# aerius-labs/paillier-halo2

Hardware: AMD Instinct MI355X
Metric: Paillier-encrypt proofs/s (2048-bit n, k=17); MSM achieved HBM GB/s vs peak (higher is better)
Workload: dtype u32 limbs (29-bit reduced radix, 254-bit modular integers), u64 limbs (4096-bit integers)

## Files before the change

### paillier_halo2_amd/csrc/pz_quotient.hip

```cpp
#include "fp29.cuh"
#include "pz_internal.h"

static inline Fr fp_one_host() {
    static const uint64_t ONE[4] = {0xac96341c4ffffffbULL, 0x36fc76959f60cd29ULL, 0x666ea36f7879462eULL, 0x0e0a77c19a07df2fULL};
    Fr r;
    memcpy(r.v, ONE, 32);
    return r;
}
static inline Fr fr_from_u64(const uint64_t x[4]) {
    Fr r;
    memcpy(r.v, x, 32);
    return r;
}

typedef F29<FrTag> Fr29;
__device__ __forceinline__ Fr29 fr29_c261(const Fr& c) { return f29_to_261(f29_from_fp(c)); }
__device__ __forceinline__ Fr29 fr29_one256() {
    Fr29 r;
#pragma unroll
    for (int i = 0; i < 9; ++i) r.v[i] = P29<FrTag>::R256(i);
    return r;
}

struct S29 {
    u32 v[9];
};
static bool host_fr_canonical(const uint64_t c[4]) {
    static const uint64_t R[4] = {0x43e1f593f0000001ULL, 0x2833e84879b97091ULL, 0xb85045b68181585dULL, 0x30644e72e131a029ULL};
    for (int i = 3; i >= 0; --i)
        if (c[i] != R[i]) return c[i] < R[i];
    return false;
}
static S29 host_fr_shl(const uint64_t c[4], unsigned k) {
    static const uint64_t R[4] = {0x43e1f593f0000001ULL, 0x2833e84879b97091ULL, 0xb85045b68181585dULL, 0x30644e72e131a029ULL};
    uint64_t x[4] = {c[0], c[1], c[2], c[3]};
    for (unsigned t = 0; t < k; ++t) {
        for (int i = 3; i > 0; --i) x[i] = (x[i] << 1) | (x[i - 1] >> 63);
        x[0] <<= 1;
        bool ge = true;
        for (int i = 3; i >= 0; --i)
            if (x[i] != R[i]) { ge = x[i] > R[i]; break; }
        if (ge) {
            unsigned __int128 br = 0;
            for (int i = 0; i < 4; ++i) {
                const unsigned __int128 d = (unsigned __int128)x[i] - R[i] - br;
                x[i] = (uint64_t)d;
                br = (d >> 64) & 1;
            }
        }
    }
    S29 r;
    for (int i = 0; i < 9; ++i) {
        const unsigned bit = 29u * i, j = bit >> 6, o = bit & 63;
        uint64_t w = x[j] >> o;
        if (o > 35 && j + 1 < 4) w |= x[j + 1] << (64 - o);
        r.v[i] = (u32)(w & (i < 8 ? 0x1fffffffull : 0xffffffffull));
    }
    return r;
}
static void host_fr_mul(const uint64_t a[4], const uint64_t b[4], uint64_t out[4]) {
    static const uint64_t R[4] = {0x43e1f593f0000001ULL, 0x2833e84879b97091ULL, 0xb85045b68181585dULL, 0x30644e72e131a029ULL};
    const uint64_t INV = 0xc2e1f593efffffffULL;
    uint64_t t[6] = {0, 0, 0, 0, 0, 0};
    for (int i = 0; i < 4; ++i) {
        unsigned __int128 c = 0;
        for (int j = 0; j < 4; ++j) {
            c += (unsigned __int128)a[j] * b[i] + t[j];
            t[j] = (uint64_t)c;
            c >>= 64;
        }
        c += t[4];
        t[4] = (uint64_t)c;
        t[5] = (uint64_t)(c >> 64);
        const uint64_t m = t[0] * INV;
        c = ((unsigned __int128)m * R[0] + t[0]) >> 64;
        for (int j = 1; j < 4; ++j) {
            c += (unsigned __int128)m * R[j] + t[j];
            t[j - 1] = (uint64_t)c;
            c >>= 64;
        }
        c += t[4];
        t[3] = (uint64_t)c;
        t[4] = t[5] + (uint64_t)(c >> 64);
    }
    bool ge = t[4] != 0;
    if (!ge) {
        ge = true;
        for (int i = 3; i >= 0; --i)
            if (t[i] != R[i]) { ge = t[i] > R[i]; break; }
    }
    if (ge) {
        unsigned __int128 br = 0;
        for (int i = 0; i < 4; ++i) {
            const unsigned __int128 d = (unsigned __int128)t[i] - R[i] - br;
            t[i] = (uint64_t)d;
            br = (d >> 64) & 1;
        }
    }
    memcpy(out, t, 32);
}
static void host_fr_pow(const uint64_t a[4], unsigned e, uint64_t out[4]) {
    static const uint64_t ONE[4] = {0xac96341c4ffffffbULL, 0x36fc76959f60cd29ULL, 0x666ea36f7879462eULL, 0x0e0a77c19a07df2fULL};
    uint64_t acc[4], sq[4];
    memcpy(acc, ONE, 32);
    memcpy(sq, a, 32);
    for (; e; e >>= 1) {
        if (e & 1) host_fr_mul(acc, sq, acc);
        host_fr_mul(sq, sq, sq);
    }
    memcpy(out, acc, 32);
}
extern "C" int pzx_host_selftest(void) {
    static const uint64_t ONE[4] = {0xac96341c4ffffffbULL, 0x36fc76959f60cd29ULL, 0x666ea36f7879462eULL, 0x0e0a77c19a07df2fULL};
    auto limbs_of = [](const uint64_t x[4]) { return host_fr_shl(x, 0); };
    auto same = [](const S29& a, const S29& b) { return memcmp(a.v, b.v, sizeof a.v) == 0; };
    uint64_t two[4], acc[4], pw[4];
    {
        const S29 d = host_fr_shl(ONE, 1);
        unsigned __int128 carry = 0;
        memset(two, 0, sizeof two);
        for (int i = 0; i < 9; ++i) {
            const unsigned bit = 29u * i, j = bit >> 6, o = bit & 63;
            two[j] |= (uint64_t)d.v[i] << o;
            if (o > 35 && j + 1 < 4) two[j + 1] |= (uint64_t)d.v[i] >> (64 - o);
        }
        (void)carry;
    }
    if (!same(limbs_of(two), host_fr_shl(ONE, 1))) return 1;
    host_fr_mul(ONE, ONE, acc);
    if (memcmp(acc, ONE, 32)) return 2;
    memcpy(acc, ONE, 32);
    for (unsigned k = 1; k <= 300; ++k) {
        host_fr_mul(acc, two, acc);
        if (!same(limbs_of(acc), host_fr_shl(ONE, k))) return 100 + (int)k;
        if (k % 37 == 0 || k == 300) {
            host_fr_pow(two, k, pw);
            if (memcmp(pw, acc, 32)) return 1000 + (int)k;
        }
    }
    return 0;
}
extern "C" void pzx_host_fr_mul(const uint64_t a[4], const uint64_t b[4], uint64_t out[4]) { host_fr_mul(a, b, out); }
extern "C" void pzx_host_fr_pow(const uint64_t a[4], unsigned e, uint64_t out[4]) { host_fr_pow(a, e, out); }
extern "C" void pzx_host_fr_shl(const uint64_t c[4], unsigned k, uint32_t out[9]) {
    const S29 r = host_fr_shl(c, k);
    memcpy(out, r.v, sizeof r.v);
}
__device__ __forceinline__ Fr29 f29_add_s(const Fr29& a, const u32 (&b)[9]) {
    Fr29 r;
#pragma unroll
    for (int i = 0; i < 9; ++i) r.v[i] = a.v[i] + b[i];
    return r;
}

__global__ __launch_bounds__(256) void k_batch_invert(Fr* __restrict__ a, Fr* __restrict__ scratch, size_t n, size_t T,
                                                      unsigned K, Fr* __restrict__ mul_io) {
    const size_t t = (size_t)blockIdx.x * blockDim.x + threadIdx.x;
    if (t >= T) return;
    Fr29 acc = fr29_one256();
    for (unsigned j = 0; j < K; ++j) {
        const size_t i = t + (size_t)j * T;
        if (i >= n) break;
        const Fr v = fp_load<FrTag>(a + i);
        if (fp_is_zero(v)) continue;
        Fr w;
        f29_pack(acc, w.v);
        fp_store(scratch + i, w);
        acc = f29_mul(acc, f29_from_fp_shl5(v));
    }
    Fr29 inv = f29_mul(f29_inv(acc), fr29_one256());
    for (unsigned j = K; j-- > 0;) {
        const size_t i = t + (size_t)j * T;
        if (i >= n) continue;
        const Fr v = fp_load<FrTag>(a + i);
        if (fp_is_zero(v)) {
            if (mul_io) fp_store(mul_io + i, fp_zero<FrTag>());
            continue;
        }
        const Fr29 ai = f29_mul(inv, f29_load<FrTag>(scratch + i));
        if (mul_io) f29_store_product(mul_io + i, f29_mul(ai, f29_load_shl5<FrTag>(mul_io + i)));
        else f29_store_product(a + i, ai);
        inv = f29_mul(inv, f29_from_fp_shl5(v));
    }
}

int pz_batch_invert_internal(pz_ctx* ctx, Fr* d_a, size_t n, Fr* d_mul_io) {
    if (!n) return PZ_OK;
    void* scr;
    PZCHK(pz_ws_get(ctx, WS_BIG_A, n * 32, &scr));
    unsigned K = 8;
    while (K < 64 && n / (K * 2) >= 16384) K *= 2;
    while (K < 512 && n / (K * 2) >= 262144) K *= 2;
    const size_t T = pz_div_up(n, K);
    hipLaunchKernelGGL(k_batch_invert, dim3(pz_div_up(T, 256)), dim3(256), 0, ctx->stream, d_a, (Fr*)scr, n, T, K, d_mul_io);
    HIPCHK(ctx, hipGetLastError());
    return PZ_OK;
}

extern "C" int pz_fr_batch_invert_dev(pz_ctx* ctx, uint64_t* d_a, size_t n) {
    if (!ctx || (n && !d_a)) return PZ_ERR_INVALID;
    PZ_ENTER(ctx);
    return pz_batch_invert_internal(ctx, (Fr*)d_a, n, nullptr);
}

#define PP_K 16u
__global__ __launch_bounds__(256) void k_pp_local(const Fr* __restrict__ a, size_t as, size_t n, Fr* __restrict__ excl,
                                                  Fr* __restrict__ block_tot, unsigned nb) {
    __shared__ u32 s[9 * 256];
    a += (size_t)blockIdx.y * as;
    const size_t t = (size_t)blockIdx.x * 256 + threadIdx.x;
    const size_t lo = t * PP_K;
    Fr29 p = fr29_one256();
    for (unsigned j = 0; j < PP_K; ++j)
        if (lo + j < n) p = f29_mul(p, f29_load_shl5<FrTag>(a + lo + j));
    p = f29_to_261(p);
#pragma unroll
    for (int i = 0; i < 9; ++i) s[i * 256 + threadIdx.x] = p.v[i];
    __syncthreads();
    for (unsigned off = 1; off < 256; off <<= 1) {
        Fr29 u;
        if (threadIdx.x >= off) {
#pragma unroll
            for (int i = 0; i < 9; ++i) u.v[i] = s[i * 256 + threadIdx.x - off];
        }
        __syncthreads();
        if (threadIdx.x >= off) {
            p = f29_mul(u, p);
#pragma unroll
            for (int i = 0; i < 9; ++i) s[i * 256 + threadIdx.x] = p.v[i];
        }
        __syncthreads();
    }
    Fr29 e = f29_one<FrTag>();
    if (threadIdx.x) {
#pragma unroll
        for (int i = 0; i < 9; ++i) e.v[i] = s[i * 256 + threadIdx.x - 1];
    }
    Fr w;
    f29_pack(e, w.v);
    fp_store(excl + (size_t)blockIdx.y * nb * 256 + t, w);
    if (threadIdx.x == 255) f29_store_product(block_tot + (size_t)blockIdx.y * nb + blockIdx.x, f29_to_256(p));
}
__global__ void k_pp_blocks(Fr* __restrict__ block_tot, unsigned nb, size_t n_cols, Fr z0) {
    const size_t col = (size_t)blockIdx.x * blockDim.x + threadIdx.x;
    if (col >= n_cols) return;
    Fr* bt = block_tot + col * nb;
    Fr run = z0;
    for (unsigned b = 0; b < nb; ++b) {
        Fr t = fp_load<FrTag>(bt + b);
        fp_store(bt + b, run);
        run = fp_mul(run, t);
    }
}
__global__ __launch_bounds__(256) void k_pp_apply(const Fr* __restrict__ a, size_t as, size_t n, const Fr* __restrict__ excl,
                                                  const Fr* __restrict__ block_tot, unsigned nb, Fr* __restrict__ z, size_t zs) {
    a += (size_t)blockIdx.y * as;
    z += (size_t)blockIdx.y * zs;
    const size_t t = (size_t)blockIdx.x * 256 + threadIdx.x;
    const size_t lo = t * PP_K;
    if (lo >= n) return;
    Fr29 cur = f29_mul(f29_load<FrTag>(block_tot + (size_t)blockIdx.y * nb + blockIdx.x),
                       f29_load<FrTag>(excl + (size_t)blockIdx.y * nb * 256 + t));
    for (unsigned j = 0; j < PP_K && lo + j < n; ++j) {
        const Fr v = fp_load<FrTag>(a + lo + j);
        f29_store_product(z + lo + j, cur);
        cur = f29_mul(cur, f29_from_fp_shl5(v));
    }
}

int pz_prefix_product_batch_internal(pz_ctx* ctx, const Fr* d_a, size_t a_stride, size_t n_cols, size_t n, Fr z0, Fr* d_z,
                                     size_t z_stride) {
    if (!n || !n_cols) return PZ_OK;
    if (n_cols > 65535) return PZ_ERR_INVALID;
    const unsigned nb = pz_div_up(pz_div_up(n, PP_K), 256);
    void* ws;
    PZCHK(pz_ws_get(ctx, WS_BIG_B, n_cols * ((size_t)nb * 256 + nb) * 32, &ws));
    Fr* excl = (Fr*)ws;
    Fr* tot = excl + n_cols * (size_t)nb * 256;
    hipLaunchKernelGGL(k_pp_local, dim3(nb, (unsigned)n_cols), dim3(256), 0, ctx->stream, d_a, a_stride, n, excl, tot, nb);
    hipLaunchKernelGGL(k_pp_blocks, dim3(pz_div_up(n_cols, 64)), dim3(64), 0, ctx->stream, tot, nb, n_cols, z0);
    hipLaunchKernelGGL(k_pp_apply, dim3(nb, (unsigned)n_cols), dim3(256), 0, ctx->stream, d_a, a_stride, n, (const Fr*)excl,
                       (const Fr*)tot, nb, d_z, z_stride);
    HIPCHK(ctx, hipGetLastError());
    return PZ_OK;
}
int pz_prefix_product_internal(pz_ctx* ctx, const Fr* d_a, size_t n, Fr z0, Fr* d_z) {
    return pz_prefix_product_batch_internal(ctx, d_a, n, 1, n, z0, d_z, n);
}

extern "C" int pz_fr_prefix_product_dev(pz_ctx* ctx, const uint64_t* d_a, size_t n, const uint64_t z0[4], uint64_t* d_z) {
    if (!ctx || !z0 || (n && (!d_a || !d_z))) return PZ_ERR_INVALID;
    PZ_ENTER(ctx);
    return pz_prefix_product_internal(ctx, (const Fr*)d_a, n, fr_from_u64(z0), (Fr*)d_z);
}

__global__ __launch_bounds__(256) void k_perm_terms(const Fr* __restrict__ cols, size_t cs, const Fr* __restrict__ sigma,
                                                    size_t ss, unsigned m, size_t n, const Fr* __restrict__ wpow, Fr beta,
                                                    Fr gamma, Fr delta0, Fr delta, Fr* __restrict__ num,
                                                    Fr* __restrict__ den) {
    const size_t i = (size_t)blockIdx.x * blockDim.x + threadIdx.x;
    if (i >= n) return;
    const Fr29 g = fr29_c261(gamma), d = fr29_c261(delta), beta266 = f29_to_261(fr29_c261(beta));
    Fr29 nm = fr29_one256(), dn = nm;
    Fr29 bd = f29_mul(f29_mul(beta266, f29_from_fp(delta0)), f29_load_shl5<FrTag>(wpow + i));
    for (unsigned j = 0; j < m; ++j) {
        const Fr29 v = f29_add(f29_load_shl5<FrTag>(cols + (size_t)j * cs + i), g);
        const Fr29 sg = f29_load<FrTag>(sigma + (size_t)j * ss + i);
        nm = f29_mul(nm, f29_add(v, bd));
        dn = f29_mul(dn, f29_add(v, f29_mul(beta266, sg)));
        bd = f29_mul(bd, d);
    }
    f29_store<0>(num + i, nm);
    f29_store<0>(den + i, dn);
}

extern "C" int pz_permutation_product_dev(pz_ctx* ctx, const uint64_t* d_cols, size_t col_stride, const uint64_t* d_sigma,
                                          size_t sigma_stride, size_t m, uint32_t log_n, const uint64_t omega[4],
                                          const uint64_t beta[4], const uint64_t gamma[4], const uint64_t delta_start[4],
                                          const uint64_t delta[4], const uint64_t z0[4], uint64_t* d_z) {
    if (!ctx || !omega || !beta || !gamma || !delta_start || !delta || !z0 || !d_z || log_n > 26) return PZ_ERR_INVALID;
    if (m && (!d_cols || !d_sigma)) return PZ_ERR_INVALID;
    if (col_stride % 4 || sigma_stride % 4 || m > 65535) return PZ_ERR_INVALID;
    const size_t n = (size_t)1 << log_n;
    if (m > 1 && (col_stride < 4 * n || sigma_stride < 4 * n)) return PZ_ERR_INVALID;
    PZ_ENTER(ctx);
    void *wp, *ws;
    PZCHK(pz_get_pow_table(ctx, omega, n, &wp));
    PZCHK(pz_ws_get(ctx, WS_BIG_C, 2 * n * 32, &ws));
    Fr* num = (Fr*)ws;
    Fr* den = num + n;
    hipLaunchKernelGGL(k_perm_terms, dim3(pz_div_up(n, 256)), dim3(256), 0, ctx->stream, (const Fr*)d_cols, col_stride / 4,
                       (const Fr*)d_sigma, sigma_stride / 4, (unsigned)m, n, (const Fr*)wp, fr_from_u64(beta), fr_from_u64(gamma),
                       fr_from_u64(delta_start), fr_from_u64(delta), num, den);
    HIPCHK(ctx, hipGetLastError());
    PZCHK(pz_batch_invert_internal(ctx, den, n, num));
    return pz_prefix_product_internal(ctx, num, n, fr_from_u64(z0), (Fr*)d_z);
}

__global__ __launch_bounds__(256) void k_perm_terms_sets(const Fr* __restrict__ cols, size_t cs, const Fr* __restrict__ sigma,
                                                         size_t ss, unsigned m, unsigned chunk_len, size_t n,
                                                         const Fr* __restrict__ wpow, const Fr* __restrict__ dpow,
                                                         S29 beta266, S29 g, S29 d, Fr* __restrict__ num, Fr* __restrict__ den,
                                                         unsigned set0) {
    const size_t i = (size_t)blockIdx.x * blockDim.x + threadIdx.x;
    if (i >= n) return;
    const unsigned c0 = (set0 + blockIdx.y) * chunk_len, set = blockIdx.y;
    Fr29 nm = fr29_one256(), dn = nm;
    Fr29 bd = f29_mul(f29_mul_s(f29_load<FrTag>(dpow + c0), beta266.v), f29_load_shl5<FrTag>(wpow + i));
    Fr v_n = fp_load<FrTag>(cols + (size_t)c0 * cs + i), s_n = fp_load<FrTag>(sigma + (size_t)c0 * ss + i);
    for (unsigned c = c0; c < c0 + chunk_len && c < m; ++c) {
        const Fr29 v = f29_add_s(f29_from_fp_shl5(v_n), g.v);
        const Fr29 sg = f29_from_fp(s_n);
        const unsigned cn = (c + 1 < c0 + chunk_len && c + 1 < m) ? c + 1 : c;
        v_n = fp_load<FrTag>(cols + (size_t)cn * cs + i);
        s_n = fp_load<FrTag>(sigma + (size_t)cn * ss + i);
        nm = f29_mul(nm, f29_add(v, bd));
        dn = f29_mul(dn, f29_add(v, f29_mul_s(sg, beta266.v)));
        bd = f29_mul_s(bd, d.v);
    }
    f29_store_product(num + (size_t)set * n + i, nm);
    f29_store_product(den + (size_t)set * n + i, dn);
}
__global__ __launch_bounds__(256) void k_perm_chain(const Fr* __restrict__ z, size_t zs, unsigned n_sets, size_t u, Fr* __restrict__ mult) {
    __shared__ Fr s_p[256];
    const unsigned per = (n_sets + 255u) / 256u, lo = threadIdx.x * per, hi = lo + per < n_sets ? lo + per : n_sets;
    Fr p = fp_one<FrTag>();
    for (unsigned j = lo; j < hi; ++j) p = fp_mul(p, fp_load<FrTag>(z + (size_t)j * zs + u));
    s_p[threadIdx.x] = p;
    __syncthreads();
    for (unsigned off = 1; off < 256; off <<= 1) {
        Fr v = fp_one<FrTag>();
        if (threadIdx.x >= off) v = s_p[threadIdx.x - off];
        __syncthreads();
        if (threadIdx.x >= off) {
            p = fp_mul(v, p);
            s_p[threadIdx.x] = p;
        }
        __syncthreads();
    }
    Fr c = threadIdx.x ? s_p[threadIdx.x - 1] : fp_one<FrTag>();
    for (unsigned j = lo; j < hi; ++j) {
        fp_store(mult + j, c);
        c = fp_mul(c, fp_load<FrTag>(z + (size_t)j * zs + u));
    }
}
__global__ __launch_bounds__(256) void k_scale_sets(Fr* __restrict__ z, size_t zs, size_t n, const Fr* __restrict__ mult) {
    const size_t i = (size_t)blockIdx.x * blockDim.x + threadIdx.x;
    if (i >= n || blockIdx.y == 0) return;
    Fr* p = z + (size_t)blockIdx.y * zs + i;
    fp_store(p, fp_mul(fp_load<FrTag>(p), fp_load<FrTag>(mult + blockIdx.y)));
}

extern "C" int pz_permutation_product_sets_dev(pz_ctx* ctx, const uint64_t* d_cols, size_t col_stride, const uint64_t* d_sigma,
                                               size_t sigma_stride, size_t m, uint32_t chunk_len, uint32_t log_n,
                                               size_t usable_rows, const uint64_t omega[4], const uint64_t beta[4],
                                               const uint64_t gamma[4], const uint64_t delta[4], uint64_t* d_z,
                                               size_t z_stride) {
    if (!ctx || !d_cols || !d_sigma || !d_z || !omega || !beta || !gamma || !delta || m == 0 || chunk_len == 0 || log_n > 26)
        return PZ_ERR_INVALID;
    const size_t n = (size_t)1 << log_n;
    const size_t n_sets = (m + chunk_len - 1) / chunk_len;
    if (col_stride % 4 || sigma_stride % 4 || z_stride % 4 || usable_rows >= n || n_sets > 65535 || m > 0xffffffu) return PZ_ERR_INVALID;
    if ((m > 1 && (col_stride < 4 * n || sigma_stride < 4 * n)) || (n_sets > 1 && z_stride < 4 * n)) return PZ_ERR_INVALID;
    if (!host_fr_canonical(beta) || !host_fr_canonical(gamma) || !host_fr_canonical(delta)) return PZ_ERR_INVALID;
    PZ_ENTER(ctx);
    void *wp, *dp, *ws, *mu;
    PZCHK(pz_get_pow_table(ctx, omega, n, &wp));
    PZCHK(pz_get_pow_table(ctx, delta, m, &dp));
    size_t sb = ((size_t)4 << 30) / (2 * n * 32);
    if (sb < 1) sb = 1;
    if (sb > n_sets) sb = n_sets;
    PZCHK(pz_ws_get(ctx, WS_BIG_C, 2 * sb * n * 32, &ws));
    PZCHK(pz_ws_get(ctx, WS_MISC, n_sets * 32, &mu));
    Fr* num = (Fr*)ws;
    Fr* den = num + sb * n;
    for (size_t s0 = 0; s0 < n_sets; s0 += sb) {
        const size_t ns = n_sets - s0 < sb ? n_sets - s0 : sb;
        hipLaunchKernelGGL(k_perm_terms_sets, dim3(pz_div_up(n, 256), (unsigned)ns), dim3(256), 0, ctx->stream,
                           (const Fr*)d_cols, col_stride / 4, (const Fr*)d_sigma, sigma_stride / 4, (unsigned)m, (unsigned)chunk_len, n,
                           (const Fr*)wp, (const Fr*)dp, host_fr_shl(beta, 10), host_fr_shl(gamma, 5), host_fr_shl(delta, 5), num, den,
                           (unsigned)s0);
        HIPCHK(ctx, hipGetLastError());
        PZCHK(pz_batch_invert_internal(ctx, den, ns * n, num));
        PZCHK(pz_prefix_product_batch_internal(ctx, num, n, ns, n, fp_one_host(), (Fr*)d_z + s0 * (z_stride / 4), z_stride / 4));
    }
    if (n_sets > 1) {
        hipLaunchKernelGGL(k_perm_chain, dim3(1), dim3(256), 0, ctx->stream, (const Fr*)d_z, z_stride / 4, (unsigned)n_sets,
                           usable_rows, (Fr*)mu);
        hipLaunchKernelGGL(k_scale_sets, dim3(pz_div_up(n, 256), (unsigned)n_sets), dim3(256), 0, ctx->stream, (Fr*)d_z,
                           z_stride / 4, n, (const Fr*)mu);
        HIPCHK(ctx, hipGetLastError());
    }
    return PZ_OK;
}

__global__ __launch_bounds__(256) void k_quotient_gate(const Fr* __restrict__ adv, size_t as, const Fr* __restrict__ sel,
                                                       size_t ss, unsigned n_cols, size_t N, unsigned step, S29 y261,
                                                       Fr* __restrict__ h) {
    const size_t i = (size_t)blockIdx.x * blockDim.x + threadIdx.x;
    if (i >= N) return;
    const size_t i1 = (i + step) & (N - 1), i2 = (i + 2 * (size_t)step) & (N - 1), i3 = (i + 3 * (size_t)step) & (N - 1);
    Fr29 acc = f29_load<FrTag>(h + i);
    for (unsigned j = 0; j < n_cols; ++j) {
        const Fr* a = adv + (size_t)j * as;
        const Fr29 a0 = f29_load<FrTag>(a + i), a1 = f29_load<FrTag>(a + i1), a3 = f29_load<FrTag>(a + i3);
        const Fr29 a2 = f29_load_shl5<FrTag>(a + i2), sl = f29_load_shl5<FrTag>(sel + (size_t)j * ss + i);
        const Fr29 e = f29_sub<2, 29>(f29_add(a0, f29_mul(a1, a2)), a3);
        acc = f29_mul2_s(acc, y261.v, e, sl);
    }
    f29_store<0>(h + i, acc);
}

extern "C" int pz_quotient_gate_dev(pz_ctx* ctx, const uint64_t* d_adv_ext, size_t adv_stride, const uint64_t* d_sel_ext,
                                    size_t sel_stride, size_t n_cols, uint32_t log_ext, uint32_t rot_step,
                                    const uint64_t y[4], uint64_t* d_h) {
    if (!ctx || !y || !d_h || log_ext > 28 || (n_cols && (!d_adv_ext || !d_sel_ext))) return PZ_ERR_INVALID;
    if (adv_stride % 4 || sel_stride % 4 || n_cols > 0xffffffffu) return PZ_ERR_INVALID;
    const size_t N = (size_t)1 << log_ext;
    if (rot_step == 0 || rot_step >= N) return PZ_ERR_INVALID;
    if (n_cols > 1 && (adv_stride < 4 * N || sel_stride < 4 * N)) return PZ_ERR_INVALID;
    if (!host_fr_canonical(y)) return PZ_ERR_INVALID;
    if (n_cols == 0) return PZ_OK;
    PZ_ENTER(ctx);
    hipLaunchKernelGGL(k_quotient_gate, dim3(pz_div_up(N, 256)), dim3(256), 0, ctx->stream, (const Fr*)d_adv_ext,
                       adv_stride / 4, (const Fr*)d_sel_ext, sel_stride / 4, (unsigned)n_cols, N, (unsigned)rot_step,
                       host_fr_shl(y, 5), (Fr*)d_h);
    HIPCHK(ctx, hipGetLastError());
    return PZ_OK;
}

__global__ void k_vanishing_inv(Fr g, Fr w_ext, unsigned log_n, unsigned E, Fr* __restrict__ out) {
    const unsigned r = threadIdx.x;
    if (blockIdx.x || r >= E) return;
    Fr x = g;
    for (unsigned k = 0; k < r; ++k) x = fp_mul(x, w_ext);
    for (unsigned k = 0; k < log_n; ++k) x = fp_sqr(x);
    fp_store(out + r, fp_inv(fp_sub(x, fp_one<FrTag>())));
}
__global__ __launch_bounds__(256) void k_scale_periodic(Fr* __restrict__ h, size_t N, const Fr* __restrict__ tab,
                                                        unsigned mask) {
    const size_t i = (size_t)blockIdx.x * blockDim.x + threadIdx.x;
    if (i < N) fp_store(h + i, fp_mul(fp_load<FrTag>(h + i), fp_load<FrTag>(tab + (i & mask))));
}

extern "C" int pz_quotient_finish_dev(pz_ctx* ctx, uint64_t* d_h, uint32_t log_n, uint32_t log_e, const uint64_t coset_g[4],
                                      const uint64_t omega_ext[4]) {
    if (!ctx || !d_h || !coset_g || !omega_ext || log_e > 6 || log_n + log_e > 28) return PZ_ERR_INVALID;
    PZ_ENTER(ctx);
    const unsigned E = 1u << log_e;
    const size_t N = (size_t)1 << (log_n + log_e);
    void* tab;
    PZCHK(pz_ws_get(ctx, WS_MISC, E * 32, &tab));
    hipLaunchKernelGGL(k_vanishing_inv, dim3(1), dim3(64), 0, ctx->stream, fr_from_u64(coset_g), fr_from_u64(omega_ext),
                       (unsigned)log_n, E, (Fr*)tab);
    hipLaunchKernelGGL(k_scale_periodic, dim3(pz_div_up(N, 256)), dim3(256), 0, ctx->stream, (Fr*)d_h, N, (const Fr*)tab,
                       E - 1);
    HIPCHK(ctx, hipGetLastError());
    return PZ_OK;
}

__global__ __launch_bounds__(256) void k_mul_table_cols(Fr* __restrict__ a, size_t cs, size_t n, const Fr* __restrict__ tab) {
    const size_t i = (size_t)blockIdx.x * blockDim.x + threadIdx.x;
    if (i >= n) return;
    Fr* p = a + (size_t)blockIdx.y * cs + i;
    fp_store(p, fp_mul(fp_load<FrTag>(p), fp_load<FrTag>(tab + i)));
}

extern "C" int pz_fr_distribute_powers_dev(pz_ctx* ctx, uint64_t* d_a, size_t n_cols, size_t col_stride, size_t n,
                                           const uint64_t g[4], const uint64_t c[4]) {
    if (!ctx || !g || (n_cols && n && !d_a) || col_stride % 4 || (n_cols > 1 && col_stride < 4 * n)) return PZ_ERR_INVALID;
    if (n_cols == 0 || n == 0) return PZ_OK;
    if (n_cols > 65535) return PZ_ERR_INVALID;
    PZ_ENTER(ctx);
    void* tab;
    PZCHK(pz_get_pow_table(ctx, g, n, &tab, c));
    hipLaunchKernelGGL(k_mul_table_cols, dim3(pz_div_up(n, 256), (unsigned)n_cols), dim3(256), 0, ctx->stream, (Fr*)d_a,
                       col_stride / 4, n, (const Fr*)tab);
    HIPCHK(ctx, hipGetLastError());
    return PZ_OK;
}

#define KD_K 64u
__global__ __launch_bounds__(256) void k_kd_local(const Fr* __restrict__ a, size_t cs, size_t n, Fr x, Fr* __restrict__ L,
                                                  size_t n_chunks) {
    const size_t c = (size_t)blockIdx.x * blockDim.x + threadIdx.x;
    if (c >= n_chunks) return;
    const Fr* p = a + (size_t)blockIdx.y * cs;
    const size_t lo = c * KD_K, hi = (lo + KD_K < n ? lo + KD_K : n);
    Fr v = fp_zero<FrTag>();
    for (size_t i = hi; i-- > lo;) v = fp_add(fp_mul(v, x), fp_load<FrTag>(p + i));
    fp_store(L + (size_t)blockIdx.y * n_chunks + c, v);
}
__global__ __launch_bounds__(256) void k_kd_carry(Fr* __restrict__ L, size_t n_chunks, Fr x) {
    __shared__ Fr s_v[256], s_x[256];
    Fr* l = L + (size_t)blockIdx.x * n_chunks;
    Fr xk = x;
    for (unsigned s = 1; s < KD_K; s <<= 1) xk = fp_sqr(xk);
    const size_t per = (n_chunks + 255) / 256;
    const size_t lo = threadIdx.x * per, hi = lo + per < n_chunks ? lo + per : n_chunks;
    Fr V = fp_zero<FrTag>(), X = fp_one<FrTag>();
    for (size_t c = hi; c-- > lo && c < n_chunks;) {
        V = fp_add(fp_load<FrTag>(l + c), fp_mul(xk, V));
        X = fp_mul(X, xk);
    }
    s_v[threadIdx.x] = V;
    s_x[threadIdx.x] = X;
    __syncthreads();
    for (unsigned off = 1; off < 256; off <<= 1) {
        Fr v = s_v[threadIdx.x], xx = s_x[threadIdx.x];
        Fr uv = fp_zero<FrTag>(), ux = fp_one<FrTag>();
        const bool has = threadIdx.x + off < 256;
        if (has) { uv = s_v[threadIdx.x + off]; ux = s_x[threadIdx.x + off]; }
        __syncthreads();
        if (has) {
            s_v[threadIdx.x] = fp_add(v, fp_mul(xx, uv));
            s_x[threadIdx.x] = fp_mul(xx, ux);
        }
        __syncthreads();
    }
    Fr carry = threadIdx.x + 1 < 256 ? s_v[threadIdx.x + 1] : fp_zero<FrTag>();
    for (size_t c = hi; c-- > lo && c < n_chunks;) {
        Fr t = fp_load<FrTag>(l + c);
        fp_store(l + c, carry);
        carry = fp_add(t, fp_mul(xk, carry));
    }
}
__global__ __launch_bounds__(256) void k_kd_apply(const Fr* a, size_t cs, size_t n, Fr x,
                                                  const Fr* __restrict__ L, size_t n_chunks, Fr* q, size_t qs) {
    const size_t c = (size_t)blockIdx.x * blockDim.x + threadIdx.x;
    if (c >= n_chunks) return;
    const Fr* p = a + (size_t)blockIdx.y * cs;
    Fr* o = q + (size_t)blockIdx.y * qs;
    const size_t lo = c * KD_K, hi = (lo + KD_K < n ? lo + KD_K : n);
    Fr cur = fp_load<FrTag>(L + (size_t)blockIdx.y * n_chunks + c);
    for (size_t i = hi; i-- > lo;) {
        Fr ai = fp_load<FrTag>(p + i);
        fp_store(o + i, cur);
        cur = fp_add(ai, fp_mul(x, cur));
    }
}

extern "C" int pz_poly_div_linear_dev(pz_ctx* ctx, const uint64_t* d_coeffs, size_t n_cols, size_t col_stride, size_t n,
                                      const uint64_t x[4], uint64_t* d_q, size_t q_stride) {
    if (!ctx || !x || (n_cols && n && (!d_coeffs || !d_q)) || col_stride % 4 || q_stride % 4) return PZ_ERR_INVALID;
    if (n_cols > 1 && (col_stride < 4 * n || q_stride < 4 * n)) return PZ_ERR_INVALID;
    if (n_cols == 0 || n == 0) return PZ_OK;
    if (n_cols > 65535) return PZ_ERR_INVALID;
    PZ_ENTER(ctx);
    const size_t nch = pz_div_up(n, KD_K);
    void* L;
    PZCHK(pz_ws_get(ctx, WS_BIG_A, n_cols * nch * 32, &L));
    Fr xv = fr_from_u64(x);
    hipLaunchKernelGGL(k_kd_local, dim3(pz_div_up(nch, 256), (unsigned)n_cols), dim3(256), 0, ctx->stream,
                       (const Fr*)d_coeffs, col_stride / 4, n, xv, (Fr*)L, nch);
    hipLaunchKernelGGL(k_kd_carry, dim3((unsigned)n_cols), dim3(256), 0, ctx->stream, (Fr*)L, nch, xv);
    hipLaunchKernelGGL(k_kd_apply, dim3(pz_div_up(nch, 256), (unsigned)n_cols), dim3(256), 0, ctx->stream,
                       (const Fr*)d_coeffs, col_stride / 4, n, xv, (const Fr*)L, nch, (Fr*)d_q, q_stride / 4);
    HIPCHK(ctx, hipGetLastError());
    return PZ_OK;
}

struct PermQ {
    const Fr *cols, *sigma, *z, *l0, *llast, *lactive, *xpow;
    size_t cs, ss, zs, N;
    unsigned n_sets, chunk_len, m_total, step, last_rot;
    unsigned set_lo, n_sets_total, head;
    S29 y, gamma, delta, beta266;
    S29 bx266;
    S29 y_chain, y_sets;
    S29 y_sets_d;
};
template <bool SPLIT> __global__ __launch_bounds__(256) void k_quotient_permutation(PermQ q, Fr* __restrict__ h, Fr* __restrict__ hd) {
    const size_t i0 = (size_t)blockIdx.x * blockDim.x + threadIdx.x;
    const size_t half = q.N >> 1;
    if (i0 >= half) return;
    const size_t mask = q.N - 1;
    size_t row[2], i_next[2], i_last[2];
    Fr29 acc[2];
#pragma unroll
    for (int r = 0; r < 2; ++r) {
        row[r] = i0 + (r ? half : 0);
        i_next[r] = (row[r] + q.step) & mask;
        i_last[r] = (row[r] + q.N - (size_t)q.last_rot * q.step) & mask;
        acc[r] = f29_load<FrTag>(h + row[r]);
    }
#pragma unroll
    for (int r = 0; r < 2 && q.head; ++r) {
        const size_t i = row[r];
        const Fr29 one = fr29_one256();
        const Fr29 l0 = f29_load_shl5<FrTag>(q.l0 + i);
        const Fr29 z_first = f29_load<FrTag>(q.z + i);
        acc[r] = f29_mul2_s(acc[r], q.y.v, f29_sub<2, 29>(one, z_first), l0);
        {
            const Fr29 ll = f29_load_shl5<FrTag>(q.llast + i);
            const Fr zl = fp_load<FrTag>(q.z + (size_t)(q.n_sets_total - 1) * q.zs + i);
            const Fr29 z_lastset = f29_from_fp(zl);
            acc[r] = f29_mul2_s(acc[r], q.y.v, f29_sub<2, 29>(f29_mul(z_lastset, f29_from_fp_shl5(zl)), z_lastset), ll);
        }
        if (q.n_sets_total > 1) {
            Fr29 t0 = f29_sub<2, 29>(f29_load<FrTag>(q.z + q.zs + i), f29_load<FrTag>(q.z + i_last[r]));
            for (unsigned j = 2; j < q.n_sets_total; ++j) {
                const Fr29 d = f29_sub<2, 29>(f29_load<FrTag>(q.z + (size_t)j * q.zs + i), f29_load<FrTag>(q.z + (size_t)(j - 1) * q.zs + i_last[r]));
                t0 = f29_add(f29_mul_s(t0, q.y.v), d);
            }
            acc[r] = f29_mul2_s(acc[r], q.y_chain.v, t0, l0);
        }
    }
    Fr29 cur = f29_mul_s(f29_load<FrTag>(q.xpow + i0), q.bx266.v);
    unsigned c = 0;
    Fr v_n[2], s_n[2];
#pragma unroll
    for (int r = 0; r < 2; ++r) {
        v_n[r] = fp_load<FrTag>(q.cols + row[r]);
        s_n[r] = fp_load<FrTag>(q.sigma + row[r]);
    }
    Fr29 hs[2];
    for (unsigned j = 0; j < q.n_sets; ++j) {
        Fr29 left[2], right[2];
#pragma unroll
        for (int r = 0; r < 2; ++r) {
            left[r] = f29_load<FrTag>(q.z + (size_t)(q.set_lo + j) * q.zs + i_next[r]);
            right[r] = f29_load<FrTag>(q.z + (size_t)(q.set_lo + j) * q.zs + row[r]);
        }
        for (unsigned t = 0; t < q.chunk_len && c < q.m_total; ++t, ++c) {
            const unsigned cn = c + 1 < q.m_total ? c + 1 : c;
#pragma unroll
            for (int r = 0; r < 2; ++r) {
                const Fr29 v = f29_add_s(f29_from_fp_shl5(v_n[r]), q.gamma.v);
                const Fr29 sg = f29_from_fp(s_n[r]);
                v_n[r] = fp_load<FrTag>(q.cols + (size_t)cn * q.cs + row[r]);
                s_n[r] = fp_load<FrTag>(q.sigma + (size_t)cn * q.ss + row[r]);
                left[r] = f29_mul(left[r], f29_add(v, f29_mul_s(sg, q.beta266.v)));
                right[r] = f29_mul(right[r], r ? f29_sub<2, 29>(v, cur) : f29_add(v, cur));
            }
            cur = f29_mul_s(cur, q.delta.v);
        }
#pragma unroll
        for (int r = 0; r < 2; ++r) {
            const Fr29 diff = f29_sub<2, 29>(left[r], right[r]);
            hs[r] = j ? f29_add(f29_mul_s(hs[r], q.y.v), diff) : diff;
        }
    }
#pragma unroll
    for (int r = 0; r < 2; ++r) {
        if (SPLIT) {
            f29_store<0>(hd + row[r], f29_mul2_s(f29_load<FrTag>(hd + row[r]), q.y_sets_d.v, hs[r], f29_one<FrTag>()));
            acc[r] = f29_mul_s(acc[r], q.y_sets.v);
        } else {
            acc[r] = f29_mul2_s(acc[r], q.y_sets.v, hs[r], f29_load_shl5<FrTag>(q.lactive + row[r]));
        }
        f29_store<0>(h + row[r], acc[r]);
    }
}

static int quotient_permutation_launch(pz_ctx* ctx, const uint64_t* d_cols_ext, size_t col_stride, const uint64_t* d_sigma_ext,
                                       size_t sigma_stride, const uint64_t* d_z_ext, size_t z_stride, uint32_t n_sets_total,
                                       uint32_t set_lo, uint32_t n_sets, uint32_t chunk_len, uint32_t m_cols, int head, uint32_t log_ext,
                                       uint32_t rot_step, uint32_t last_rotation, const uint64_t* d_l0, const uint64_t* d_l_last,
                                       const uint64_t* d_l_active, const uint64_t beta[4], const uint64_t gamma[4],
                                       const uint64_t delta[4], const uint64_t coset_g[4], const uint64_t omega_ext[4],
                                       const uint64_t y[4], uint64_t* d_h, uint64_t* d_hd) {
    if (!ctx || !d_cols_ext || !d_sigma_ext || !d_z_ext || !d_l0 || !d_l_last || (!d_l_active && !d_hd) || !beta || !gamma || !delta ||
        !coset_g || !omega_ext || !y || !d_h || d_h == d_hd)
        return PZ_ERR_INVALID;
    if (log_ext > 28 || log_ext == 0 || n_sets == 0 || chunk_len == 0 || m_cols == 0 || col_stride % 4 || sigma_stride % 4 || z_stride % 4)
        return PZ_ERR_INVALID;
    if (n_sets_total == 0 || (size_t)set_lo + n_sets > n_sets_total) return PZ_ERR_INVALID;
    const size_t N = (size_t)1 << log_ext;
    if ((size_t)n_sets * chunk_len < m_cols || (size_t)(n_sets - 1) * chunk_len >= m_cols) return PZ_ERR_INVALID;
    if (set_lo + n_sets < n_sets_total && (size_t)n_sets * chunk_len != m_cols) return PZ_ERR_INVALID;
    if (rot_step == 0 || rot_step >= N || (size_t)last_rotation * rot_step >= N) return PZ_ERR_INVALID;
    if ((m_cols > 1 && (col_stride < 4 * N || sigma_stride < 4 * N)) || (n_sets_total > 1 && z_stride < 4 * N)) return PZ_ERR_INVALID;
    if (!host_fr_canonical(beta) || !host_fr_canonical(gamma) || !host_fr_canonical(delta) || !host_fr_canonical(y)) return PZ_ERR_INVALID;
    PZ_ENTER(ctx);
    PermQ q;
    q.cols = (const Fr*)d_cols_ext; q.sigma = (const Fr*)d_sigma_ext; q.z = (const Fr*)d_z_ext;
    q.l0 = (const Fr*)d_l0; q.llast = (const Fr*)d_l_last; q.lactive = (const Fr*)d_l_active;
    q.cs = col_stride / 4; q.ss = sigma_stride / 4; q.zs = z_stride / 4; q.N = N;
    q.n_sets = n_sets; q.chunk_len = chunk_len; q.m_total = m_cols; q.step = rot_step; q.last_rot = last_rotation;
    q.set_lo = set_lo; q.n_sets_total = n_sets_total; q.head = head ? 1u : 0u;
    q.beta266 = host_fr_shl(beta, 10); q.gamma = host_fr_shl(gamma, 5); q.delta = host_fr_shl(delta, 5); q.y = host_fr_shl(y, 5);
    uint64_t yp[4], bx[4];
    host_fr_pow(delta, set_lo * chunk_len, bx);
    host_fr_mul(bx, beta, bx);
    q.bx266 = host_fr_shl(bx, 10);
    host_fr_pow(y, n_sets_total - 1, yp);
    q.y_chain = host_fr_shl(yp, 5);
    host_fr_pow(y, n_sets, yp);
    q.y_sets = host_fr_shl(yp, 5);
    host_fr_pow(y, n_sets + (head ? 2 + (n_sets_total > 1 ? n_sets_total - 1 : 0) : 0), yp);
    q.y_sets_d = host_fr_shl(yp, 5);
    void* xp;
    PZCHK(pz_get_pow_table(ctx, omega_ext, N, &xp, coset_g));
    q.xpow = (const Fr*)xp;
// ... 264 lines not shown
```

Measured before the change: 1.458.

## Fold cross-set permutation chaining into prefix-product apply pass

Result: slower. 1.434 (-1.6%).

```diff
diff --git a/paillier_halo2_amd/csrc/pz_quotient.hip b/paillier_halo2_amd/csrc/pz_quotient.hip
--- a/paillier_halo2_amd/csrc/pz_quotient.hip
+++ b/paillier_halo2_amd/csrc/pz_quotient.hip
@@ -1,3 +1,5 @@
+#include <cstdlib>
+
 #include "fp29.cuh"
 #include "pz_internal.h"
 
@@ -252,8 +254,45 @@
         run = fp_mul(run, t);
     }
 }
+__global__ __launch_bounds__(256) void k_perm_chain(const Fr* __restrict__ z, size_t zs, unsigned n_sets, size_t u, Fr* __restrict__ mult,
+                                                    Fr* __restrict__ carry, unsigned has_carry) {
+    __shared__ Fr s_p[256];
+    const unsigned per = (n_sets + 255u) / 256u, lo = threadIdx.x * per, hi = lo + per < n_sets ? lo + per : n_sets;
+    const Fr cin = has_carry ? fp_load<FrTag>(carry) : fp_one<FrTag>();
+    Fr p = fp_one<FrTag>();
+    for (unsigned j = lo; j < hi; ++j) p = fp_mul(p, fp_load<FrTag>(z + (size_t)j * zs + u));
+    s_p[threadIdx.x] = p;
+    __syncthreads();
+    for (unsigned off = 1; off < 256; off <<= 1) {
+        Fr v = fp_one<FrTag>();
+        if (threadIdx.x >= off) v = s_p[threadIdx.x - off];
+        __syncthreads();
+        if (threadIdx.x >= off) {
+            p = fp_mul(v, p);
+            s_p[threadIdx.x] = p;
+        }
+        __syncthreads();
+    }
+    Fr c = threadIdx.x ? fp_mul(cin, s_p[threadIdx.x - 1]) : cin;
+    for (unsigned j = lo; j < hi; ++j) {
+        fp_store(mult + j, c);
+        c = fp_mul(c, fp_load<FrTag>(z + (size_t)j * zs + u));
+    }
+    if (threadIdx.x == 255) fp_store(carry, fp_mul(cin, s_p[255]));
+}
+__global__ __launch_bounds__(64) void k_pp_row(const Fr* __restrict__ a, size_t as, size_t u, const Fr* __restrict__ excl,
+                                               const Fr* __restrict__ block_tot, unsigned nb, size_t n_cols,
+                                               Fr* __restrict__ out) {
+    const size_t col = (size_t)blockIdx.x * blockDim.x + threadIdx.x;
+    if (col >= n_cols) return;
+    const size_t t = u / PP_K;
+    Fr29 cur = f29_mul(f29_load<FrTag>(block_tot + col * nb + t / 256), f29_load<FrTag>(excl + col * nb * 256 + t));
+    for (size_t i = t * PP_K; i < u; ++i) cur = f29_mul(cur, f29_load_shl5<FrTag>(a + col * as + i));
+    f29_store_product(out + col, cur);
+}
 __global__ __launch_bounds__(256) void k_pp_apply(const Fr* __restrict__ a, size_t as, size_t n, const Fr* __restrict__ excl,
-                                                  const Fr* __restrict__ block_tot, unsigned nb, Fr* __restrict__ z, size_t zs) {
+                                                  const Fr* __restrict__ block_tot, unsigned nb, Fr* __restrict__ z, size_t zs,
+                                                  const Fr* __restrict__ mu) {
     a += (size_t)blockIdx.y * as;
     z += (size_t)blockIdx.y * zs;
     const size_t t = (size_t)blockIdx.x * 256 + threadIdx.x;
@@ -261,6 +300,7 @@
     if (lo >= n) return;
     Fr29 cur = f29_mul(f29_load<FrTag>(block_tot + (size_t)blockIdx.y * nb + blockIdx.x),
                        f29_load<FrTag>(excl + (size_t)blockIdx.y * nb * 256 + t));
+    if (mu) cur = f29_mul(cur, f29_load_shl5<FrTag>(mu + blockIdx.y));
     for (unsigned j = 0; j < PP_K && lo + j < n; ++j) {
         const Fr v = fp_load<FrTag>(a + lo + j);
         f29_store_product(z + lo + j, cur);
@@ -268,8 +308,21 @@
     }
 }
 
+struct PpChain {
+    size_t u;
+    Fr* at_u;
+    Fr* mu;
+    Fr* carry;
+    unsigned has_carry;
+};
+static int pz_prefix_product_batch_chained(pz_ctx* ctx, const Fr* d_a, size_t a_stride, size_t n_cols, size_t n, Fr z0, Fr* d_z,
+                                           size_t z_stride, const PpChain* chain);
 int pz_prefix_product_batch_internal(pz_ctx* ctx, const Fr* d_a, size_t a_stride, size_t n_cols, size_t n, Fr z0, Fr* d_z,
                                      size_t z_stride) {
+    return pz_prefix_product_batch_chained(ctx, d_a, a_stride, n_cols, n, z0, d_z, z_stride, nullptr);
+}
+static int pz_prefix_product_batch_chained(pz_ctx* ctx, const Fr* d_a, size_t a_stride, size_t n_cols, size_t n, Fr z0, Fr* d_z,
+                                           size_t z_stride, const PpChain* chain) {
     if (!n || !n_cols) return PZ_OK;
     if (n_cols > 65535) return PZ_ERR_INVALID;
     const unsigned nb = pz_div_up(pz_div_up(n, PP_K), 256);
@@ -279,8 +332,14 @@
     Fr* tot = excl + n_cols * (size_t)nb * 256;
     hipLaunchKernelGGL(k_pp_local, dim3(nb, (unsigned)n_cols), dim3(256), 0, ctx->stream, d_a, a_stride, n, excl, tot, nb);
     hipLaunchKernelGGL(k_pp_blocks, dim3(pz_div_up(n_cols, 64)), dim3(64), 0, ctx->stream, tot, nb, n_cols, z0);
+    if (chain) {
+        hipLaunchKernelGGL(k_pp_row, dim3(pz_div_up(n_cols, 64)), dim3(64), 0, ctx->stream, d_a, a_stride, chain->u, (const Fr*)excl,
+                           (const Fr*)tot, nb, n_cols, chain->at_u);
+        hipLaunchKernelGGL(k_perm_chain, dim3(1), dim3(256), 0, ctx->stream, (const Fr*)chain->at_u, (size_t)1, (unsigned)n_cols,
+                           (size_t)0, chain->mu, chain->carry, chain->has_carry);
+    }
     hipLaunchKernelGGL(k_pp_apply, dim3(nb, (unsigned)n_cols), dim3(256), 0, ctx->stream, d_a, a_stride, n, (const Fr*)excl,
-                       (const Fr*)tot, nb, d_z, z_stride);
+                       (const Fr*)tot, nb, d_z, z_stride, chain ? (const Fr*)chain->mu : (const Fr*)nullptr);
     HIPCHK(ctx, hipGetLastError());
     return PZ_OK;
 }
@@ -361,34 +420,14 @@
     f29_store_product(num + (size_t)set * n + i, nm);
     f29_store_product(den + (size_t)set * n + i, dn);
 }
-__global__ __launch_bounds__(256) void k_perm_chain(const Fr* __restrict__ z, size_t zs, unsigned n_sets, size_t u, Fr* __restrict__ mult) {
-    __shared__ Fr s_p[256];
-    const unsigned per = (n_sets + 255u) / 256u, lo = threadIdx.x * per, hi = lo + per < n_sets ? lo + per : n_sets;
-    Fr p = fp_one<FrTag>();
-    for (unsigned j = lo; j < hi; ++j) p = fp_mul(p, fp_load<FrTag>(z + (size_t)j * zs + u));
-    s_p[threadIdx.x] = p;
-    __syncthreads();
-    for (unsigned off = 1; off < 256; off <<= 1) {
-        Fr v = fp_one<FrTag>();
-        if (threadIdx.x >= off) v = s_p[threadIdx.x - off];
-        __syncthreads();
-        if (threadIdx.x >= off) {
-            p = fp_mul(v, p);
-            s_p[threadIdx.x] = p;
-        }
-        __syncthreads();
-    }
-    Fr c = threadIdx.x ? s_p[threadIdx.x - 1] : fp_one<FrTag>();
-    for (unsigned j = lo; j < hi; ++j) {
-        fp_store(mult + j, c);
-        c = fp_mul(c, fp_load<FrTag>(z + (size_t)j * zs + u));
-    }
-}
-__global__ __launch_bounds__(256) void k_scale_sets(Fr* __restrict__ z, size_t zs, size_t n, const Fr* __restrict__ mult) {
-    const size_t i = (size_t)blockIdx.x * blockDim.x + threadIdx.x;
-    if (i >= n || blockIdx.y == 0) return;
-    Fr* p = z + (size_t)blockIdx.y * zs + i;
-    fp_store(p, fp_mul(fp_load<FrTag>(p), fp_load<FrTag>(mult + blockIdx.y)));
+static size_t perm_set_batch(size_t n, size_t n_sets) {
+    size_t sb = ((size_t)4 << 30) / (2 * n * 32);
+    const char* e = getenv("PZ_PERM_SET_BATCH");
+    const long env = e ? atol(e) : 0;
+    if (env > 0 && (size_t)env < sb) sb = (size_t)env;
+    if (sb < 1) sb = 1;
+    if (sb > n_sets) sb = n_sets;
+    return sb;
 }
 
 extern "C" int pz_permutation_product_sets_dev(pz_ctx* ctx, const uint64_t* d_cols, size_t col_stride, const uint64_t* d_sigma,
@@ -407,13 +446,12 @@
     void *wp, *dp, *ws, *mu;
     PZCHK(pz_get_pow_table(ctx, omega, n, &wp));
     PZCHK(pz_get_pow_table(ctx, delta, m, &dp));
-    size_t sb = ((size_t)4 << 30) / (2 * n * 32);
-    if (sb < 1) sb = 1;
-    if (sb > n_sets) sb = n_sets;
+    const size_t sb = perm_set_batch(n, n_sets);
     PZCHK(pz_ws_get(ctx, WS_BIG_C, 2 * sb * n * 32, &ws));
-    PZCHK(pz_ws_get(ctx, WS_MISC, n_sets * 32, &mu));
+    PZCHK(pz_ws_get(ctx, WS_MISC, (2 * sb + 1) * 32, &mu));
     Fr* num = (Fr*)ws;
     Fr* den = num + sb * n;
+    PpChain chain = {usable_rows, (Fr*)mu + sb, (Fr*)mu, (Fr*)mu + 2 * sb, 0u};
     for (size_t s0 = 0; s0 < n_sets; s0 += sb) {
         const size_t ns = n_sets - s0 < sb ? n_sets - s0 : sb;
         hipLaunchKernelGGL(k_perm_terms_sets, dim3(pz_div_up(n, 256), (unsigned)ns), dim3(256), 0, ctx->stream,
@@ -422,14 +460,9 @@
                            (unsigned)s0);
         HIPCHK(ctx, hipGetLastError());
         PZCHK(pz_batch_invert_internal(ctx, den, ns * n, num));
-        PZCHK(pz_prefix_product_batch_internal(ctx, num, n, ns, n, fp_one_host(), (Fr*)d_z + s0 * (z_stride / 4), z_stride / 4));
-    }
-    if (n_sets > 1) {
-        hipLaunchKernelGGL(k_perm_chain, dim3(1), dim3(256), 0, ctx->stream, (const Fr*)d_z, z_stride / 4, (unsigned)n_sets,
-                           usable_rows, (Fr*)mu);
-        hipLaunchKernelGGL(k_scale_sets, dim3(pz_div_up(n, 256), (unsigned)n_sets), dim3(256), 0, ctx->stream, (Fr*)d_z,
-                           z_stride / 4, n, (const Fr*)mu);
-        HIPCHK(ctx, hipGetLastError());
+        chain.has_carry = s0 != 0;
+        PZCHK(pz_prefix_product_batch_chained(ctx, num, n, ns, n, fp_one_host(), (Fr*)d_z + s0 * (z_stride / 4), z_stride / 4,
+                                              n_sets > 1 ? &chain : nullptr));
     }
     return PZ_OK;
 }
```
